# wang-q/gams

Measured on AMD Instinct MI355X. Metric: GC windows/s (size 100, step 10), higher is better.
Workload: dtype u8; 1 GPU; Atha-shaped synthetic genome (119667750 bp, piece 500000): wave size 100 step 10 lag 100 threshold 3 influence 1, peaks compacted on device; 3 batch(es) resident per GPU, steps rotate over them; batches_per_gpu=3, resident_bytes_per_gpu=358913250, passes_in_flight=3, tapered_launches=off in the timed region (passes in flight), clock_ramp_steps=4992, device=gfx950:sramecc+:xnack-, parallelism=ctg-sharded x1, no collective on the data path, collectives=none (one rank)

## Files before the change

### gams_amd/_lib.py

```python
import ctypes as C
import os

import numpy as np

_HERE = os.path.dirname(os.path.abspath(__file__))
SO_PATH = os.path.join(_HERE, "libgams_gpu.so")

OK, EINVAL, ENODEV, ENOMEM, EHIP, ESHORT, EUNSUPPORTED, ESTATE = range(8)
WAVE_PEAKS, WAVE_DENSE = 1, 2
WAVE_INPUT_AUTO, WAVE_INPUT_BYTES, WAVE_INPUT_PLANE = 0, 1, 2
WAVE_BODY_AUTO, WAVE_BODY_WIDE, WAVE_BODY_NARROW = 0, 1, 2
GC_BODY_AUTO, GC_BODY_PORTABLE, GC_BODY_AVX2 = 0, 1, 2
SW_GC, SW_COUNT = 1, 2


class GamsError(RuntimeError):
    def __init__(self, code, msg):
        super().__init__(f"gams_gpu error {code}: {msg}")
        self.code = code


class WaveParams(C.Structure):
    _fields_ = [("size", C.c_int32), ("step", C.c_int32), ("lag", C.c_uint32),
                ("threshold", C.c_float), ("influence", C.c_float)]


class GenParams(C.Structure):
    _fields_ = [("piece", C.c_int32), ("fill", C.c_int32), ("min_len", C.c_int32)]


GEN_CTG_DTYPE = np.dtype([("chr", np.uint32), ("serial", np.uint32), ("chr_start", np.int32), ("chr_end", np.int32)])
PEAK_DTYPE = np.dtype([("ctg", np.uint32), ("window", np.uint32), ("gc_count", np.uint32),
                       ("signal", np.int32)])
SW_ROW_DTYPE = np.dtype([("feature", np.uint32), ("type", np.int32), ("distance", np.int32),
                         ("start", np.int32), ("end", np.int32), ("gc_content", np.float32),
                         ("gc_mean", np.float32), ("gc_stddev", np.float32), ("gc_cv", np.float32)])

_VP = C.c_void_p
_PP = C.POINTER(C.c_void_p)
PROTOTYPES = {
    "gams_gpu_create": (C.c_int, [C.c_int, _PP]),
    "gams_gpu_destroy": (None, [_VP]),
    "gams_gpu_last_error": (C.c_char_p, [_VP]),
    "gams_gpu_device_info": (C.c_int, [_VP, C.c_char_p, C.c_size_t, C.POINTER(C.c_int32), C.POINTER(C.c_uint64)]),
    "gams_gpu_release_cached": (C.c_int, [_VP, _VP]),
    "gams_gpu_sync": (C.c_int, [_VP]),
    "gams_gpu_timer_start": (C.c_int, [_VP]),
    "gams_gpu_timer_stop": (C.c_int, [_VP, C.POINTER(C.c_float)]),
    "gams_gpu_last_kernel_ms": (C.c_int, [_VP, C.POINTER(C.c_float)]),
    "gams_gpu_last_stage_ms": (C.c_int, [_VP, _VP, C.c_uint32, C.POINTER(C.c_uint32)]),
    "gams_gpu_host_alloc": (C.c_int, [_VP, C.c_uint64, _PP]),
    "gams_gpu_host_free": (None, [_VP, _VP]),
    "gams_window_count": (C.c_int64, [C.c_int64, C.c_int32, C.c_int32]),
    "gams_seqset_create": (C.c_int, [_VP, C.c_uint32, _VP, _PP]),
    "gams_seqset_upload": (C.c_int, [_VP, _VP, C.c_uint32, _VP]),
    "gams_seqset_upload_all": (C.c_int, [_VP, _VP, _VP]),
    "gams_seqset_layout": (C.c_int, [_VP, _VP, _VP, C.POINTER(C.c_uint64)]),
    "gams_seqset_upload_image": (C.c_int, [_VP, _VP, _VP, C.c_uint64, C.c_uint64]),
    "gams_seqset_upload_ranges": (C.c_int, [_VP, _VP, _VP, _VP, C.c_uint64, C.c_uint64]),
    "gams_gc_plane": (C.c_int, [_VP, C.c_uint64, _VP]),
    "gams_gc_plane_with": (C.c_int, [_VP, C.c_uint64, _VP, C.c_int]),
    "gams_wave_plan_set_input": (C.c_int, [_VP, _VP, C.c_int]),
    "gams_wave_plan_last_input": (C.c_int, [_VP, _VP, C.POINTER(C.c_int)]),
    "gams_wave_plan_set_body": (C.c_int, [_VP, _VP, C.c_int]),
    "gams_wave_plan_last_body": (C.c_int, [_VP, _VP, C.POINTER(C.c_int)]),
    "gams_seqset_download": (C.c_int, [_VP, _VP, C.c_uint32, _VP, _VP]),
    "gams_seqset_destroy": (None, [_VP, _VP]),
    "gams_wave_plan_create": (C.c_int, [_VP, _VP, C.POINTER(WaveParams), C.c_uint32, _PP]),
    "gams_wave_plan_destroy": (None, [_VP, _VP]),
    "gams_wave_total_windows": (C.c_uint64, [_VP]),
    "gams_wave_ctg_windows": (C.c_uint32, [_VP, C.c_uint32]),
    "gams_wave_run_n": (C.c_int, [_VP, _VP, C.c_uint32]),
    "gams_wave_plan_set_depth": (C.c_int, [_VP, _VP, C.c_uint32]),
    "gams_wave_plan_select": (C.c_int, [_VP, _VP, C.c_uint32]),
    "gams_wave_plan_set_lane": (C.c_int, [_VP, _VP, C.c_uint32]),
    "gams_wave_plan_set_taper": (C.c_int, [_VP, _VP, C.c_int]),
    "gams_wave_plan_set_taper_shape": (C.c_int, [_VP, _VP, C.c_int, C.c_int]),
    "gams_wave_plan_set_queue_threads": (C.c_int, [_VP, _VP, C.c_uint32]),
    "gams_wave_plan_kernel_name": (C.c_int, [_VP, _VP, C.c_char_p, C.c_size_t]),
    "gams_wave_plan_set_pipelined": (C.c_int, [_VP, _VP, C.c_int]),
    "gams_wave_run": (C.c_int, [_VP, _VP]),
    "gams_wave_peaks": (C.c_int, [_VP, _VP, _PP, C.POINTER(C.c_uint64)]),
    "gams_wave_rows_setup": (C.c_int, [_VP, _VP, C.POINTER(C.c_char_p), _VP, C.c_float]),
    "gams_wave_rows_begin": (C.c_int, [_VP, _VP]),
    "gams_wave_rows_end": (C.c_int, [_VP, _VP, _PP, C.POINTER(C.c_uint64), _PP]),
    "gams_wave_signal_text": (C.c_int, [_VP, _VP, C.POINTER(C.c_char_p), _VP, _PP, C.POINTER(C.c_uint64), _PP]),
    "gams_wave_dense": (C.c_int, [_VP, _VP, C.c_uint32, _VP, _VP]),
    "gams_wave_plan_set_tile": (C.c_int, [_VP, _VP, C.c_uint32]),
    "gams_wave_plan_set_threads": (C.c_int, [_VP, _VP, C.c_uint32]),
    "gams_wave_plan_settled": (C.c_int, [_VP, _VP, C.POINTER(C.c_uint32), C.POINTER(C.c_int)]),
    "gams_wave_exact_count": (C.c_int, [_VP, _VP, C.POINTER(C.c_uint64)]),
    "gams_wave_plan_set_guard": (C.c_int, [_VP, _VP, C.c_float, C.c_int]),
    "gams_wave_plan_set_stamps": (C.c_int, [_VP, _VP, C.c_int]),
    "gams_wave_stamps": (C.c_int, [_VP, _VP, C.POINTER(C.c_double), C.POINTER(C.c_uint64)]),
    "gams_wave_stamps_raw": (C.c_int, [_VP, _VP, _VP, C.c_uint64]),
    "gams_gpu_wave": (C.c_int, [_VP, _VP, C.c_uint32, C.POINTER(WaveParams), _VP, _VP, C.POINTER(C.c_uint32)]),
    "gams_gpu_sw": (C.c_int, [_VP, _VP, C.c_uint32, C.c_int32, _VP, _VP, C.c_uint32, C.c_int32, C.c_int32,
                              C.c_int32, _VP, C.c_uint64, C.POINTER(C.c_uint64)]),
# ... 69 lines not shown
```

### gams_amd/csrc/wave.hip

```cpp

#include "common.hpp"

#include <algorithm>
#include <atomic>
#include <cmath>
#include <condition_variable>
#include <memory>
#include <mutex>
#include <thread>
#include <type_traits>

#include "wave_kernels.hpp"
#include "wave_repair.hpp"
#include "wave_rows.hpp"
#include "wave_select.hpp"

using WaveFastFn = void (*)(const WaveTile *, const uint8_t *, WaveArgs);
using WaveTileFn = void (*)(WaveArgs);
#define WAVE_X_PAIR(W, SIZE, STEP, LAG, NTH) \
    {wave_fast_kernel<W, SIZE, STEP, LAG, false, NTH>, wave_fast_kernel<W, SIZE, STEP, LAG, true, NTH>},
static const WaveFastFn kWaveFastFn[kWaveFastCount][2] = {WAVE_FAST_INSTANCES(WAVE_X_PAIR)};
#undef WAVE_X_PAIR
static const WaveFastFn kWaveTaperFn[2] = {wave_fast_taper_kernel<100, 10, 100, false>, wave_fast_taper_kernel<100, 10, 100, true>};
static const WaveFastFn kWaveNarrowFn = wave_fast_narrow_kernel;
static const WaveTileFn kWaveTileFn[2][2] = {{wave_tile_kernel<uint8_t, false>, wave_tile_kernel<uint8_t, true>},
                                             {wave_tile_kernel<uint16_t, false>, wave_tile_kernel<uint16_t, true>}};


struct WaveRows {
    uint32_t dmax = 0, max_name = 0;
    Kept<uint8_t> arena;
    RowTabsDev tabs;
    unsigned long long *d_words = nullptr;
    Kept<uint8_t> tmp;
    uint64_t cap = 0;
    Kept<char> d_text;
    Kept<char> h_text{true};
    Kept<unsigned long long> h_words{true};
    uint64_t copy_bytes = 0;
    bool use_graph = true;
    struct RowGraphKey {
        const void *dense, *tmp, *text, *h_text, *peaks, *tile_cnt, *tile_off;
        uint64_t dense_cap, cap, copy_bytes;
        uint32_t tile_cap, nt;
    };
    struct RowGraph {
        hipGraphExec_t exec = nullptr;
        RowGraphKey key{};
    } graph[gams_gpu::kMaxWays];
    uint64_t copied = 0;
    uint64_t last_bytes = 0;
    hipEvent_t done = nullptr;
    bool begun = false;
    void release(gams_gpu_t *h) { gams_free_all(h, arena, tmp, d_text, h_text, h_words); }
};

struct WaveSig {
// ... 53 lines not shown
    Way way[gams_gpu::kMaxWays];
    uint32_t depth = 1;
    uint32_t lane = 0;
    int taper_req = -1;
    int taper4_pct = 25, taper8_pct = 50;
    uint32_t queue_threads = gams_gpu::kMaxWays;
    uint32_t last_way = 0;
    uint32_t sel_age = 0;
    hipEvent_t ready = nullptr;
    Kept<gams_peak_t> h_peaks{true};
    uint32_t tile_cap = 0, tile_cap_req = 0;
    uint32_t tw_req = 0;
    uint32_t nth_req = 0;
    Kept<gams_peak_t> d_dense;
    uint64_t dense_cap() const { return d_dense.cap / sizeof(gams_peak_t); }
    uint64_t run_idx = 0;
    int8_t *d_const_sig = nullptr;
    unsigned long long *d_stamps = nullptr;
    unsigned long long *d_tile_off = nullptr;
    Kept<uint8_t> arena_fixed, arena_geom;
    bool ran = false;
    struct Launcher *launcher[gams_gpu::kMaxWays - 1] = {};
    bool pipelined = false;
    float g0 = 0, g1 = 0, g2 = 0, g3 = 0;
    float sq[6] = {0, 0, 0, 0, 0, 0};
    WaveRows *rows = nullptr;
    WaveSig *sigtext = nullptr;
    float guard_safety = 1.5f;
    bool guard_exact = false;
    int input_req = GAMS_WAVE_INPUT_AUTO;
    std::atomic<int> last_input{GAMS_WAVE_INPUT_BYTES};
    int body_req = GAMS_WAVE_BODY_AUTO;
    std::atomic<int> last_body{GAMS_WAVE_BODY_WIDE};
    void release(gams_gpu_t *h) {
        if (rows) rows->release(h);
        if (sigtext) sigtext->release(h);
        gams_free_all(h, arena_fixed, arena_geom, d_jtiles, d_dense, h_peaks);
        for (Way &w : way) w.release(h);
    }
};
static void wave_launcher_stop(gams_wave_plan_t *p);


namespace {

constexpr uint32_t kCounterRing = 128;
constexpr size_t kSlotWords = (size_t)kShards * kShardWords;
constexpr uint32_t kOffOneGroup = 32768;

struct Chain {
    hipStream_t st;
    hipGraph_t graph = nullptr;
    hipGraphNode_t last = nullptr;
    hipError_t err = hipSuccess;
    void kernel(const void *fn, unsigned grid, unsigned block, void **args) {
        if (err != hipSuccess) return;
        if (!graph) {
            err = hipLaunchKernel(fn, dim3(grid), dim3(block), args, 0, st);
            return;
        }
        hipKernelNodeParams kp{};
        kp.func = const_cast<void *>(fn);
        kp.gridDim = dim3(grid);
        kp.blockDim = dim3(block);
        kp.sharedMemBytes = 0;
        kp.kernelParams = args;
// ... 82 lines not shown
            p->tiles.push_back(WaveTile{c, w, n, 0u, p->ctgs[c].seq_off, p->ctgs[c].win_base});
    }
}

void wave_fill_tiles_tapered(gams_wave_plan_t *p, uint32_t slots) {
    const gams_wave_params_t &q = p->prm;
    const uint32_t tw12 = 256u * 12u - q.lag - 1u, tw8 = 256u * 8u - q.lag - 1u, tw4 = 256u * 4u - q.lag - 1u;
    const uint64_t T = p->total_windows;
    const int k4 = p->taper4_pct, k8 = p->taper8_pct;
    const uint64_t x4 = std::min<uint64_t>((uint64_t)slots * k4 / 100 * tw4, T * 8 / 100);
    const uint64_t y8 = std::min<uint64_t>((uint64_t)slots * k8 / 100 * tw8, T * 17 / 100);
    p->tiles.clear();
    for (uint32_t c = 0; c < p->set->n_ctg; ++c) {
        const uint32_t n = p->ctgs[c].n_win;
        const uint64_t after = T - p->ctgs[c].win_base;
        const uint32_t w_kind = after <= x4 ? 4u : after <= x4 + y8 ? 8u : 12u;
        const uint32_t tw = w_kind == 4u ? tw4 : w_kind == 8u ? tw8 : tw12;
        for (uint32_t w = 0; w < n; w += tw)
            p->tiles.push_back(WaveTile{c, w, n, w_kind, p->ctgs[c].seq_off, p->ctgs[c].win_base});
    }
}

int wave_build_geometry(gams_gpu_t *h, gams_wave_plan_t *p, uint32_t tw_req) {
    const WaveSelectIn in{p->prm,  p->flags,   p->serial,    p->repair, p->depth,     p->total_windows,
                          tw_req,  p->nth_req, p->taper_req, h->cus,    p->set->bytes};
    WaveSelection s;
    if (!wave_select(in, s)) return gams_fail(h, GAMS_ESTATE, "wave: the instance list lacks the selected kernel");
    p->sel = s;
    p->fast_fn = s.entry < 0 ? nullptr : s.taper ? kWaveTaperFn[s.nt] : kWaveFastFn[s.entry][s.nt];
    p->tile_fn = s.family == kWaveFamTile ? kWaveTileFn[s.k16][s.wide] : nullptr;
    if (p->fast_fn) GAMS_HIP(h, gams_lds_attr(h, reinterpret_cast<const void *>(p->fast_fn), s.lds_bytes));
    if (p->tile_fn) GAMS_HIP(h, gams_lds_attr(h, reinterpret_cast<const void *>(p->tile_fn), s.lds_bytes));
    p->body = wave_select_body(in, s);
    if (p->body.narrow) GAMS_HIP(h, gams_lds_attr(h, reinterpret_cast<const void *>(kWaveNarrowFn), p->body.lds_bytes));
    if (s.taper)
        wave_fill_tiles_tapered(p, wave_slots(h->cus));
    else
        wave_fill_tiles(p);
    return GAMS_OK;
}

void wave_set_band(gams_wave_plan_t *p) {
    float g[4];
    wave_guard_band(p->prm, (double)p->guard_safety, p->guard_exact, g);
    p->g0 = g[0];
    p->g1 = g[1];
    p->g2 = g[2];
    p->g3 = g[3];
    wave_squared_band(p->prm, g, p->sq);
}

hipStream_t wave_stream(gams_gpu_t *h, const gams_wave_plan_t *p, uint32_t k) {
    const uint32_t si = (p->lane + k) % (uint32_t)gams_gpu::kMaxWays;
    return si == 0 ? h->compute : h->aux[si - 1];
}

gams_wave_plan::Way &wave_read_way(gams_wave_plan_t *p) {
    return p->way[(p->last_way + p->depth - (p->sel_age % p->depth)) % p->depth];
}
uint32_t wave_read_way_index(const gams_wave_plan_t *p) {
    return (p->last_way + p->depth - (p->sel_age % p->depth)) % p->depth;
}

int wave_sync_ways(gams_gpu_t *h, gams_wave_plan_t *p) {
    for (uint32_t k = 0; k < p->depth; ++k) GAMS_HIP(h, hipStreamSynchronize(wave_stream(h, p, k)));
    return GAMS_OK;
}
// ... 428 lines not shown
    a.tile_cap = p->tile_cap;
    a.counters = w.d_counters + kSlotWords * slot;
    a.const_sig = p->d_const_sig;
    a.stamps = p->d_stamps;
    a.tile_cnt = w.d_tile_cnt;
    a.dense_cnt = w.d_dense_cnt;
    a.dense_sig = w.d_dense_sig;
    return a;
}

static int wave_pass_on_way(gams_gpu_t *h, gams_wave_plan_t *p, uint32_t k) {
    gams_wave_plan::Way &w = p->way[k];
    hipStream_t st = wave_stream(h, p, k);
    h->reader_epoch.fetch_add(1, std::memory_order_relaxed);
    if (st == h->compute) {
        int wrc = gams_seqset_wait_uploads(h, p->set);
        if (wrc != GAMS_OK) return wrc;
    } else if (w.seen_upload != p->set->upload_gen && p->set->uploaded) {
        GAMS_HIP(h, hipStreamWaitEvent(st, p->set->uploaded, 0));
    }
    w.seen_upload = p->set->upload_gen;
    if (!w.seen_ready) {
        GAMS_HIP(h, hipStreamWaitEvent(st, p->ready, 0));
        w.seen_ready = true;
    }
    const uint32_t slot = (uint32_t)(w.runs % kCounterRing);
    if (slot == 0 && w.runs > 0)
        GAMS_HIP(h, hipMemsetAsync(w.d_counters, 0, kCounterRing * kSlotWords * sizeof(unsigned long long), st));
    ++w.runs;
    w.last_ring = slot;
    if (p->pipelined && !w.done) GAMS_HIP(h, hipEventCreateWithFlags(&w.done, hipEventDisableTiming));
    if (p->tiles.empty()) {
        p->last_body.store(GAMS_WAVE_BODY_WIDE, std::memory_order_relaxed);
        if (p->pipelined) GAMS_HIP(h, hipEventRecord(w.done, st));
        return GAMS_OK;
    }
    const gams_wave_params_t &q = p->prm;
    const bool fast_tile = p->fast_fn != nullptr;
    const bool plane_fit = fast_tile && p->set->plane_ok && p->set->d_plane != nullptr;
    if (p->input_req == GAMS_WAVE_INPUT_PLANE && !plane_fit)
        return gams_fail(h, GAMS_ESTATE, fast_tile ? "wave: the seqset's G/C plane is stale" : "wave: this plan's kernels read the sequence bytes, not the G/C plane");
    const bool use_plane = plane_fit && (p->input_req != GAMS_WAVE_INPUT_BYTES || !p->set->have_bytes);
    if (!use_plane && !p->set->have_bytes)
        return gams_fail(h, GAMS_ESTATE, "wave: the seqset holds the G/C plane only and this plan needs the sequence bytes");
    if (p->input_req == GAMS_WAVE_INPUT_BYTES && use_plane)
        return gams_fail(h, GAMS_ESTATE, "wave: the seqset holds the G/C plane only, the bytes were asked for");
    p->last_input.store(use_plane ? GAMS_WAVE_INPUT_PLANE : GAMS_WAVE_INPUT_BYTES, std::memory_order_relaxed);
    const bool narrow_fit = use_plane && p->body.narrow;
    if (p->body_req == GAMS_WAVE_BODY_NARROW && !narrow_fit)
        return gams_fail(h, GAMS_ESTATE, p->body.narrow ? "wave: the narrow body reads the G/C plane, this pass reads the bytes"
                                                        : "wave: this plan has no narrow body");
    const bool narrow = narrow_fit && p->body_req != GAMS_WAVE_BODY_WIDE;
    p->last_body.store(narrow ? GAMS_WAVE_BODY_NARROW : GAMS_WAVE_BODY_WIDE, std::memory_order_relaxed);
    const WaveArgs a = wave_args(p, w, slot, use_plane);
    const unsigned nt = (unsigned)p->tiles.size();
    if (p->sel.direct) {
        const uint64_t total = p->total_windows;
        const unsigned blocks = (unsigned)((total + 255) / 256);
        hipLaunchKernelGGL(wave_direct_count_kernel, dim3(blocks), dim3(256), 0, st, p->set->d_seq, p->d_ctgs,
                           p->set->n_ctg, total, (uint32_t)q.size, (uint32_t)q.step, w.d_dense_cnt);
        GAMS_HIP(h, hipGetLastError());
        if (!p->serial || p->repair) {
            hipLaunchKernelGGL(wave_direct_signal_kernel, dim3(blocks), dim3(256), 0, st, p->d_ctgs, p->set->n_ctg,
                               total, w.d_dense_cnt, w.d_dense_sig, q.lag, q.threshold, (float)q.size,
                               q.lag < 2 ? 1u : 0u);
            GAMS_HIP(h, hipGetLastError());
        }
    } else if (narrow) {
        hipLaunchKernelGGL(kWaveNarrowFn, dim3(nt), dim3(p->body.nth), p->body.lds_bytes, st, a.tiles, a.seq, a);
        GAMS_HIP(h, hipGetLastError());
    } else if (p->fast_fn) {
        hipLaunchKernelGGL(p->fast_fn, dim3(nt), dim3(p->sel.nth), p->sel.lds_bytes, st, a.tiles, a.seq, a);
        GAMS_HIP(h, hipGetLastError());
    } else {
        hipLaunchKernelGGL(p->tile_fn, dim3(nt), dim3(256), p->sel.lds_bytes, st, a);
        GAMS_HIP(h, hipGetLastError());
    }
    int rc = GAMS_OK;
    if (p->sel.direct && !p->serial) {
        rc = wave_compact_dense(h, p, k, st);
        if (rc != GAMS_OK) return rc;
    }
    if (p->repair) {
        w.jac_sweeps = 0;
        w.jac_settled = false;
        w.jac_serial = false;
        rc = wave_jac_sweeps(h, p, k, kJacFirstBatch, true);
        if (rc != GAMS_OK) return rc;
    } else if (p->serial) {
        rc = wave_serial_recurrence(h, p, k, st, w.d_filtered);
        if (rc == GAMS_OK) rc = wave_compact_dense(h, p, k, st);
        if (rc != GAMS_OK) return rc;
    }
    if (p->pipelined) GAMS_HIP(h, hipEventRecord(w.done, st));
    return GAMS_OK;
}

static int wave_wait_last_run(gams_gpu_t *h, gams_wave_plan_t *p) {
    gams_wave_plan::Way &w = wave_read_way(p);
    if (p->pipelined && w.done)
        GAMS_HIP(h, hipEventSynchronize(w.done));
    else
        GAMS_HIP(h, hipStreamSynchronize(wave_stream(h, p, wave_read_way_index(p))));
    return GAMS_OK;
}

int gams_wave_plan_set_input(gams_gpu_t *h, gams_wave_plan_t *p, int mode) {
    if (!h || !p) return gams_fail(h, GAMS_EINVAL, "wave_plan_set_input: null argument");
    if (mode != GAMS_WAVE_INPUT_AUTO && mode != GAMS_WAVE_INPUT_BYTES && mode != GAMS_WAVE_INPUT_PLANE)
        return gams_fail(h, GAMS_EINVAL, "wave_plan_set_input: mode is 0 (auto), 1 (bytes) or 2 (plane)");
    p->input_req = mode;
    return GAMS_OK;
}

int gams_wave_plan_last_input(gams_gpu_t *h, gams_wave_plan_t *p, int *input) {
    if (!h || !p || !input) return gams_fail(h, GAMS_EINVAL, "wave_plan_last_input: null argument");
    if (!p->ran) return gams_fail(h, GAMS_ESTATE, "wave_plan_last_input: no run yet");
    *input = p->last_input.load(std::memory_order_relaxed);
    return GAMS_OK;
}

int gams_wave_plan_set_body(gams_gpu_t *h, gams_wave_plan_t *p, int mode) {
    if (!h || !p) return gams_fail(h, GAMS_EINVAL, "wave_plan_set_body: null argument");
    if (mode != GAMS_WAVE_BODY_AUTO && mode != GAMS_WAVE_BODY_WIDE && mode != GAMS_WAVE_BODY_NARROW)
        return gams_fail(h, GAMS_EINVAL, "wave_plan_set_body: mode is 0 (auto), 1 (wide) or 2 (narrow)");
    p->body_req = mode;
    return GAMS_OK;
}

int gams_wave_plan_last_body(gams_gpu_t *h, gams_wave_plan_t *p, int *body) {
    if (!h || !p || !body) return gams_fail(h, GAMS_EINVAL, "wave_plan_last_body: null argument");
    if (!p->ran) return gams_fail(h, GAMS_ESTATE, "wave_plan_last_body: no run yet");
    *body = p->last_body.load(std::memory_order_relaxed);
    return GAMS_OK;
}

int gams_wave_plan_set_pipelined(gams_gpu_t *h, gams_wave_plan_t *p, int enable) {
    if (!h || !p) return gams_fail(h, GAMS_EINVAL, "wave_plan_set_pipelined: null argument");
    p->pipelined = enable != 0;
    return GAMS_OK;
}

int gams_wave_run(gams_gpu_t *h, gams_wave_plan_t *p) {
    if (!h || !p) return gams_fail(h, GAMS_EINVAL, "wave_run: null argument");
    GAMS_HIP(h, hipSetDevice(h->device));
    const uint32_t k = (uint32_t)(p->run_idx % p->depth);
    int rc = wave_pass_on_way(h, p, k);
    if (rc != GAMS_OK) return rc;
    ++p->run_idx;
    p->last_way = k;
    p->sel_age = 0;
    p->ran = true;
    return GAMS_OK;
}

struct Launcher {
    std::thread th;
    std::mutex mu;
    std::condition_variable cv;
    bool armed = false, quit = false, finished = true;
    std::atomic<int> go{0};
    gams_gpu_t *h = nullptr;
    gams_wave_plan_t *p = nullptr;
    uint64_t first = 0;
    uint32_t rest = 0;
    uint32_t share = 0, shares = 1;
// ... 792 lines not shown
```

### gams_amd/csrc/wave_kernels.hpp

```cpp
#pragma once

#include "common.hpp"

#include <type_traits>

namespace {

struct WaveCtgDev {
    uint64_t seq_off;
    uint64_t win_base;
    uint32_t len;
    uint32_t n_win;
};

struct WaveTile {
    uint32_t ctg;
    uint32_t w0;
    uint32_t n_win;
    uint32_t pad;
    uint64_t seq_off;
    uint64_t win_base;
};

constexpr uint32_t kShards = 128;
// ... 855 lines not shown
template <int W, int SIZE, int STEP, int LAG, bool NT, int NTH = 256>
__device__ __forceinline__ void wave_fast_pick(const WaveTile tl, const uint8_t *const seq_p, const WaveArgs &a) {
    if (a.plane != nullptr)
        wave_fast_tile<W, SIZE, STEP, LAG, NT, NTH, true>(tl, seq_p, a);
    else
        wave_fast_tile<W, SIZE, STEP, LAG, NT, NTH, false>(tl, seq_p, a);
}

template <int W, int SIZE, int STEP, int LAG, bool NT, int NTH = 256>
__global__ __launch_bounds__(NTH, 8) void wave_fast_kernel(const WaveTile *const tiles_p, const uint8_t *const seq_p,
                                                           const WaveArgs a) {
    const WaveTile tl = tiles_p[blockIdx.x];
    wave_fast_pick<W, SIZE, STEP, LAG, NT, NTH>(tl, seq_p, a);
}

template <int SIZE, int STEP, int LAG, bool NT>
__global__ __launch_bounds__(256, 8) void wave_fast_taper_kernel(const WaveTile *const tiles_p,
                                                                 const uint8_t *const seq_p, const WaveArgs a) {
    const WaveTile tl = tiles_p[blockIdx.x];
    if (tl.pad == 12u)
        wave_fast_pick<12, SIZE, STEP, LAG, NT>(tl, seq_p, a);
    else if (tl.pad == 8u)
        wave_fast_pick<8, SIZE, STEP, LAG, NT>(tl, seq_p, a);
    else
        wave_fast_pick<4, SIZE, STEP, LAG, NT>(tl, seq_p, a);
}

__global__ __launch_bounds__(128, 8) void wave_fast_narrow_kernel(const WaveTile *const tiles_p, const uint8_t *const seq_p,
                                                                  const WaveArgs a) {
    const WaveTile tl = tiles_p[blockIdx.x];
    wave_fast_tile<24, 100, 10, 100, false, 128, true>(tl, seq_p, a);
}

__device__ __forceinline__ uint32_t wave_ctg_of(const WaveCtgDev *ctgs, uint32_t n_ctg, uint64_t g) {
    uint32_t lo = 0, hi = n_ctg;
    while (hi - lo > 1u) {
        const uint32_t mid = (lo + hi) >> 1;
        if (ctgs[mid].win_base <= g)
            lo = mid;
        else
            hi = mid;
    }
    return lo;
}

__global__ __launch_bounds__(256) void wave_direct_count_kernel(const uint8_t *seq, const WaveCtgDev *ctgs,
                                                                 uint32_t n_ctg, uint64_t total, uint32_t size,
                                                                 uint32_t step, uint32_t *dense_cnt) {
    const uint64_t g = (uint64_t)blockIdx.x * 256u + threadIdx.x;
    if (g >= total) return;
    const WaveCtgDev cg = ctgs[wave_ctg_of(ctgs, n_ctg, g)];
    const uint64_t b0 = cg.seq_off + (g - cg.win_base) * (uint64_t)step, b1 = b0 + size;
    uint32_t cnt = 0;
    for (uint64_t a = b0 & ~(uint64_t)3; a < b1; a += 4) {
        uint32_t f = gc_flags(*reinterpret_cast<const uint32_t *>(seq + a));
        if (a < b0) f &= ~0u << (8u * (uint32_t)(b0 - a));
        if (a + 4 > b1) f &= ~0u >> (8u * (uint32_t)(a + 4 - b1));
        cnt += (uint32_t)__popc(f);
    }
    dense_cnt[g] = cnt;
}

__global__ __launch_bounds__(256) void wave_direct_signal_kernel(const WaveCtgDev *ctgs, uint32_t n_ctg,
                                                                  uint64_t total, const uint32_t *dense_cnt,
                                                                  int8_t *dense_sig, uint32_t lag, float thr,
                                                                  float fsize, uint32_t no_signal) {
// ... 310 lines not shown
```

### gams_amd/csrc/wave_select.hpp

```cpp
#pragma once

#include <algorithm>
#include <cmath>
#include <cstddef>
#include <cstdint>
#include <cstdio>

#include "../../include/gams_gpu.h"

namespace {

#define WAVE_FAST_INSTANCES(X)                                                                        \
    X(20, 0, 0, 0, 256) X(12, 0, 0, 0, 256) X(8, 0, 0, 0, 256) X(4, 0, 0, 0, 256)                     \
    X(28, 100, 1, 100, 64) X(28, 100, 1, 100, 128) X(28, 100, 1, 100, 256)                            \
    X(20, 100, 1, 100, 256) X(12, 100, 1, 100, 256)                                                   \
    X(12, 100, 10, 100, 64) X(12, 100, 10, 100, 128) X(12, 100, 10, 100, 256)                         \
    X(8, 100, 10, 100, 256) X(4, 100, 10, 100, 256)                                                   \
    X(4, 100, 5, 0, 256) X(8, 100, 5, 0, 256) X(12, 100, 5, 0, 256)                                   \
    X(4, 100, 10, 0, 256) X(8, 100, 10, 0, 256) X(12, 100, 10, 0, 256)                                \
    X(4, 100, 20, 0, 256) X(8, 100, 20, 0, 256) X(12, 100, 20, 0, 256)                                \
    X(20, 100, 1, 0, 256)                                                                             \
    X(20, 100, 5, 0, 64) X(20, 100, 5, 0, 128) X(20, 100, 5, 0, 256)                                  \
    X(28, 100, 1, 0, 64) X(28, 100, 1, 0, 128) X(28, 100, 1, 0, 256)

// ... 171 lines not shown
    out.family = kWaveFamTile;
    out.tw = tw;
    out.max_win = tw + q.lag + 1;
    out.max_chunks = (uint32_t)((halo_bytes + (uint64_t)tw * q.step + 15) / 16) + 1;
    out.k16 = q.size > 255;
    const uint64_t ns = (uint64_t)q.lag * (uint64_t)q.size;
    const uint64_t q2max = (uint64_t)(out.max_win + 1) * (uint64_t)q.size * (uint64_t)q.size;
    out.wide = !(ns <= 65535 && q2max < (1ull << 32));
    out.lds_bytes = wave_lds_bytes(out.max_chunks, out.max_win, out.wide, out.k16);
    if (out.lds_bytes > 160 * 1024) return go_direct();
    return true;
}

struct WaveBody {
    bool narrow = false;
    uint32_t nth = 0, w = 0;
    size_t lds_bytes = 0;
};
constexpr int kWaveNarrowW = 24, kWaveNarrowNth = 128;

inline WaveBody wave_select_body(const WaveSelectIn &in, const WaveSelection &sel) {
    WaveBody b;
    if (sel.family != kWaveFamFast || sel.entry < 0 || sel.taper) return b;
    const WaveInstance &e = kWaveFast[sel.entry];
    if (!(e.w == 12 && e.size == 100 && e.step == 10 && e.lag == 100 && e.nth == 256)) return b;
    if ((in.flags & GAMS_WAVE_DENSE) || in.serial || in.nth_req != 0) return b;
    b.narrow = true;
    b.nth = (uint32_t)kWaveNarrowNth;
    b.w = (uint32_t)kWaveNarrowW;
    b.lds_bytes = wave_fast_lds_bytes(sel.max_chunks, b.w, (uint32_t)e.lag, false, b.nth);
    return b;
}

inline void wave_selection_name(const WaveSelection &s, char *buf, size_t n) {
    const char *nt = s.nt ? "true" : "false";
    if (s.direct)
        std::snprintf(buf, n, "wave_direct_count_kernel + wave_direct_signal_kernel");
    else if (s.taper)
        std::snprintf(buf, n, "wave_fast_taper_kernel<100, 10, 100, %s>", nt);
    else if (s.entry >= 0) {
        const WaveInstance &e = kWaveFast[s.entry];
        std::snprintf(buf, n, "wave_fast_kernel<%d, %d, %d, %d, %s, %d>", e.w, e.size, e.step, e.lag, nt, e.nth);
    } else
        std::snprintf(buf, n, "wave_tile_kernel<%s, %s>", s.k16 ? "unsigned short" : "unsigned char", s.wide ? "true" : "false");
}

}
```

### gams_amd/engine.py

```python
import ctypes as C

import numpy as np

from . import _lib
from ._lib import GamsError, WaveParams, PEAK_DTYPE, SW_ROW_DTYPE, WAVE_PEAKS, WAVE_DENSE


def _u8(buf):
    if isinstance(buf, np.ndarray):
        return np.ascontiguousarray(buf, dtype=np.uint8)
    return np.frombuffer(buf, dtype=np.uint8)


class Engine:

    def __init__(self, device=0, lib=None):
        self.lib = lib if lib is not None else _lib.load()
        h = C.c_void_p()
        rc = self.lib.gams_gpu_create(device, C.byref(h))
        if rc != _lib.OK:
            raise GamsError(rc, "gams_gpu_create failed (no HIP device?)")
        self.h = h
        self.device = device

# ... 245 lines not shown
            return int(nb.value)
        offs = np.frombuffer((C.c_uint64 * (n + 1)).from_address(off.value), np.uint64).copy()
        return (C.string_at(txt.value, nb.value) if nb.value else b""), offs

    def set_taper_shape(self, pct4, pct8=None):
        if pct8 is None:
            pct4, pct8 = divmod(int(pct4), 1000)
        self.eng.check(self.eng.lib.gams_wave_plan_set_taper_shape(self.eng.h, self.p, pct4, pct8))

    def set_queue_threads(self, n):
        self.eng.check(self.eng.lib.gams_wave_plan_set_queue_threads(self.eng.h, self.p, n))

    def kernel_name(self):
        buf = C.create_string_buffer(160)
        self.eng.check(self.eng.lib.gams_wave_plan_kernel_name(self.eng.h, self.p, buf, len(buf)))
        return buf.value.decode()

    def set_input(self, mode):
        self.eng.check(self.eng.lib.gams_wave_plan_set_input(self.eng.h, self.p, mode))

    def last_input(self):
        v = C.c_int()
        self.eng.check(self.eng.lib.gams_wave_plan_last_input(self.eng.h, self.p, C.byref(v)))
        return int(v.value)

    def set_body(self, mode):
        self.eng.check(self.eng.lib.gams_wave_plan_set_body(self.eng.h, self.p, mode))

    def last_body(self):
        v = C.c_int()
        self.eng.check(self.eng.lib.gams_wave_plan_last_body(self.eng.h, self.p, C.byref(v)))
        return int(v.value)

    def select(self, age):
        self.eng.check(self.eng.lib.gams_wave_plan_select(self.eng.h, self.p, age))

    def run_n(self, n):
        self.eng.check(self.eng.lib.gams_wave_run_n(self.eng.h, self.p, n))

    def run(self):
        self.eng.check(self.eng.lib.gams_wave_run(self.eng.h, self.p))

    def peaks(self):
        ptr, n = C.c_void_p(), C.c_uint64()
        self.eng.check(self.eng.lib.gams_wave_peaks(self.eng.h, self.p, C.byref(ptr), C.byref(n)))
        if n.value == 0:
            return np.zeros(0, PEAK_DTYPE)
        buf = (C.c_char * (n.value * PEAK_DTYPE.itemsize)).from_address(ptr.value)
        return np.frombuffer(buf, dtype=PEAK_DTYPE).copy()

    def dense(self, i):
        n = self.ctg_windows(i)
        cnt = np.zeros(max(n, 1), np.uint32)
        sig = np.zeros(max(n, 1), np.int8)
        self.eng.check(self.eng.lib.gams_wave_dense(self.eng.h, self.p, i, cnt.ctypes.data, sig.ctypes.data))
        return cnt[:n], sig[:n]

    def stamps(self):
        self.eng.check(self.eng.lib.gams_wave_plan_set_stamps(self.eng.h, self.p, 1))
        self.run()
        m = (C.c_double * 8)()
        span = C.c_uint64()
        self.eng.check(self.eng.lib.gams_wave_stamps(self.eng.h, self.p, m, C.byref(span)))
        self.eng.check(self.eng.lib.gams_wave_plan_set_stamps(self.eng.h, self.p, 0))
        span_ticks, sum_ticks = span.value >> 32, (span.value & 0xffffffff) * 16
        info = dict(clock_ghz=m[7], span_us=span_ticks / 100.0,
# ... 22 lines not shown
```

### include/gams_gpu_diag.h

```cpp
#ifndef GAMS_GPU_DIAG_H
#define GAMS_GPU_DIAG_H

#include "gams_gpu.h"

#ifdef __cplusplus
extern "C" {
#endif

int gams_gpu_timer_start(gams_gpu_t *h);
int gams_gpu_timer_stop(gams_gpu_t *h, float *ms);
int gams_gpu_last_kernel_ms(gams_gpu_t *h, float *ms);

int gams_gpu_last_stage_ms(gams_gpu_t *h, float *ms, uint32_t cap, uint32_t *n);

int gams_wave_plan_set_taper(gams_gpu_t *h, gams_wave_plan_t *plan, int mode);
int gams_wave_plan_set_taper_shape(gams_gpu_t *h, gams_wave_plan_t *plan, int pct4, int pct8);
int gams_wave_plan_set_queue_threads(gams_gpu_t *h, gams_wave_plan_t *plan, uint32_t n);
int gams_wave_plan_kernel_name(gams_gpu_t *h, gams_wave_plan_t *plan, char *buf, size_t n);
int gams_wave_plan_settled(gams_gpu_t *h, gams_wave_plan_t *plan, uint32_t *sweeps, int *serial);

int gams_wave_plan_set_tile(gams_gpu_t *h, gams_wave_plan_t *p, uint32_t tile_windows);
int gams_wave_plan_set_threads(gams_gpu_t *h, gams_wave_plan_t *p, uint32_t threads);
int gams_wave_exact_count(gams_gpu_t *h, gams_wave_plan_t *p, uint64_t *n_exact);
int gams_wave_plan_set_guard(gams_gpu_t *h, gams_wave_plan_t *p, float safety, int all_exact);
int gams_wave_plan_set_stamps(gams_gpu_t *h, gams_wave_plan_t *p, int enable);
int gams_wave_stamps(gams_gpu_t *h, gams_wave_plan_t *p, double *mean_cycles ,
                     uint64_t *span_cycles);
int gams_wave_stamps_raw(gams_gpu_t *h, gams_wave_plan_t *p, uint64_t *out, uint64_t n_words);

#define GAMS_WAVE_INPUT_AUTO 0
#define GAMS_WAVE_INPUT_BYTES 1
#define GAMS_WAVE_INPUT_PLANE 2
int gams_wave_plan_set_input(gams_gpu_t *h, gams_wave_plan_t *p, int mode);
int gams_wave_plan_last_input(gams_gpu_t *h, gams_wave_plan_t *p, int *input);
#define GAMS_WAVE_BODY_AUTO 0
#define GAMS_WAVE_BODY_WIDE 1
#define GAMS_WAVE_BODY_NARROW 2
int gams_wave_plan_set_body(gams_gpu_t *h, gams_wave_plan_t *p, int mode);
int gams_wave_plan_last_body(gams_gpu_t *h, gams_wave_plan_t *p, int *body);
#define GAMS_GC_BODY_AUTO 0
#define GAMS_GC_BODY_PORTABLE 1
#define GAMS_GC_BODY_AVX2 2
int gams_gc_plane_with(const uint8_t *seq, uint64_t n, uint8_t *plane, int body);

#ifdef __cplusplus
}
#endif
#endif
```

Baseline: 1427 billion windows/s.

## Add a one-wavefront narrow wave kernel and make it the default cut

Adds a new narrow-body kernel that runs each tile with a single 64-thread wavefront. Each thread owns 48 windows, and the lag sums are built from per-thread partial sums held in LDS. Plan setup and launch now choose between the existing two-wave narrow kernel and this cut, with one-wave as the auto default. The aim is to cut block-level synchronisation and cross-wave overhead, and to raise the number of resident blocks per CU. The cost is more serial work per thread. The tile width the kernel assumes must also match the geometry the plan already built.

Result: faster. 1557 billion windows/s (median of 6 runs) (+9.1%).

```diff
diff --git a/gams_amd/_lib.py b/gams_amd/_lib.py
--- a/gams_amd/_lib.py
+++ b/gams_amd/_lib.py
@@ -10,6 +10,7 @@
 WAVE_PEAKS, WAVE_DENSE = 1, 2
 WAVE_INPUT_AUTO, WAVE_INPUT_BYTES, WAVE_INPUT_PLANE = 0, 1, 2
 WAVE_BODY_AUTO, WAVE_BODY_WIDE, WAVE_BODY_NARROW = 0, 1, 2
+WAVE_CUT_AUTO, WAVE_CUT_TWO_WAVES, WAVE_CUT_ONE_WAVE = 0, 1, 2
 GC_BODY_AUTO, GC_BODY_PORTABLE, GC_BODY_AVX2 = 0, 1, 2
 SW_GC, SW_COUNT = 1, 2
 
@@ -64,6 +65,8 @@
     "gams_wave_plan_last_input": (C.c_int, [_VP, _VP, C.POINTER(C.c_int)]),
     "gams_wave_plan_set_body": (C.c_int, [_VP, _VP, C.c_int]),
     "gams_wave_plan_last_body": (C.c_int, [_VP, _VP, C.POINTER(C.c_int)]),
+    "gams_wave_plan_set_cut": (C.c_int, [_VP, _VP, C.c_int]),
+    "gams_wave_plan_last_cut": (C.c_int, [_VP, _VP, C.POINTER(C.c_int)]),
     "gams_seqset_download": (C.c_int, [_VP, _VP, C.c_uint32, _VP, _VP]),
     "gams_seqset_destroy": (None, [_VP, _VP]),
     "gams_wave_plan_create": (C.c_int, [_VP, _VP, C.POINTER(WaveParams), C.c_uint32, _PP]),
diff --git a/gams_amd/csrc/wave.hip b/gams_amd/csrc/wave.hip
--- a/gams_amd/csrc/wave.hip
+++ b/gams_amd/csrc/wave.hip
@@ -23,6 +23,10 @@
 #undef WAVE_X_PAIR
 static const WaveFastFn kWaveTaperFn[2] = {wave_fast_taper_kernel<100, 10, 100, false>, wave_fast_taper_kernel<100, 10, 100, true>};
 static const WaveFastFn kWaveNarrowFn = wave_fast_narrow_kernel;
+static const WaveFastFn kWaveOneWaveFn = wave_fast_onewave_kernel;
+static_assert(kOneWaveLds == wave_onewave_lds_bytes() && kOneWavePad == kWaveOneWavePad, "the one-wave carve of wave_select.hpp is the kernel's");
+static_assert(kWaveCutAuto == GAMS_WAVE_CUT_AUTO && kWaveCutTwoWaves == GAMS_WAVE_CUT_TWO_WAVES && kWaveCutOneWave == GAMS_WAVE_CUT_ONE_WAVE,
+              "wave_select.hpp names the cuts as gams_gpu_diag.h does");
 static const WaveTileFn kWaveTileFn[2][2] = {{wave_tile_kernel<uint8_t, false>, wave_tile_kernel<uint8_t, true>},
                                              {wave_tile_kernel<uint16_t, false>, wave_tile_kernel<uint16_t, true>}};
 
@@ -142,6 +146,8 @@
     std::atomic<int> last_input{GAMS_WAVE_INPUT_BYTES};
     int body_req = GAMS_WAVE_BODY_AUTO;
     std::atomic<int> last_body{GAMS_WAVE_BODY_WIDE};
+    int cut_req = GAMS_WAVE_CUT_AUTO;
+    std::atomic<int> last_cut{GAMS_WAVE_CUT_AUTO};
     void release(gams_gpu_t *h) {
         if (rows) rows->release(h);
         if (sigtext) sigtext->release(h);
@@ -290,7 +296,10 @@
     if (p->fast_fn) GAMS_HIP(h, gams_lds_attr(h, reinterpret_cast<const void *>(p->fast_fn), s.lds_bytes));
     if (p->tile_fn) GAMS_HIP(h, gams_lds_attr(h, reinterpret_cast<const void *>(p->tile_fn), s.lds_bytes));
     p->body = wave_select_body(in, s);
-    if (p->body.narrow) GAMS_HIP(h, gams_lds_attr(h, reinterpret_cast<const void *>(kWaveNarrowFn), p->body.lds_bytes));
+    if (p->body.narrow) {
+        GAMS_HIP(h, gams_lds_attr(h, reinterpret_cast<const void *>(kWaveNarrowFn), p->body.lds_bytes));
+        GAMS_HIP(h, gams_lds_attr(h, reinterpret_cast<const void *>(kWaveOneWaveFn), wave_onewave_lds_bytes()));
+    }
     if (s.taper)
         wave_fill_tiles_tapered(p, wave_slots(h->cus));
     else
@@ -785,6 +794,7 @@
     if (p->pipelined && !w.done) GAMS_HIP(h, hipEventCreateWithFlags(&w.done, hipEventDisableTiming));
     if (p->tiles.empty()) {
         p->last_body.store(GAMS_WAVE_BODY_WIDE, std::memory_order_relaxed);
+        p->last_cut.store(GAMS_WAVE_CUT_AUTO, std::memory_order_relaxed);
         if (p->pipelined) GAMS_HIP(h, hipEventRecord(w.done, st));
         return GAMS_OK;
     }
@@ -805,6 +815,11 @@
                                                         : "wave: this plan has no narrow body");
     const bool narrow = narrow_fit && p->body_req != GAMS_WAVE_BODY_WIDE;
     p->last_body.store(narrow ? GAMS_WAVE_BODY_NARROW : GAMS_WAVE_BODY_WIDE, std::memory_order_relaxed);
+    if (p->cut_req == GAMS_WAVE_CUT_ONE_WAVE && !narrow_fit)
+        return gams_fail(h, GAMS_ESTATE, p->body.narrow ? "wave: the one-wave cut reads the G/C plane, this pass reads the bytes"
+                                                        : "wave: this plan has no narrow body to cut");
+    const WaveCut cut = narrow ? wave_select_cut(p->body, p->cut_req) : WaveCut{};
+    p->last_cut.store(cut.cut, std::memory_order_relaxed);
     const WaveArgs a = wave_args(p, w, slot, use_plane);
     const unsigned nt = (unsigned)p->tiles.size();
     if (p->sel.direct) {
@@ -820,7 +835,8 @@
             GAMS_HIP(h, hipGetLastError());
         }
     } else if (narrow) {
-        hipLaunchKernelGGL(kWaveNarrowFn, dim3(nt), dim3(p->body.nth), p->body.lds_bytes, st, a.tiles, a.seq, a);
+        const WaveFastFn cut_fn = cut.cut == GAMS_WAVE_CUT_ONE_WAVE ? kWaveOneWaveFn : kWaveNarrowFn;
+        hipLaunchKernelGGL(cut_fn, dim3(nt), dim3(cut.nth), cut.lds_bytes, st, a.tiles, a.seq, a);
         GAMS_HIP(h, hipGetLastError());
     } else if (p->fast_fn) {
         hipLaunchKernelGGL(p->fast_fn, dim3(nt), dim3(p->sel.nth), p->sel.lds_bytes, st, a.tiles, a.seq, a);
@@ -885,6 +901,21 @@
     if (!h || !p || !body) return gams_fail(h, GAMS_EINVAL, "wave_plan_last_body: null argument");
     if (!p->ran) return gams_fail(h, GAMS_ESTATE, "wave_plan_last_body: no run yet");
     *body = p->last_body.load(std::memory_order_relaxed);
+    return GAMS_OK;
+}
+
+int gams_wave_plan_set_cut(gams_gpu_t *h, gams_wave_plan_t *p, int mode) {
+    if (!h || !p) return gams_fail(h, GAMS_EINVAL, "wave_plan_set_cut: null argument");
+    if (mode != GAMS_WAVE_CUT_AUTO && mode != GAMS_WAVE_CUT_TWO_WAVES && mode != GAMS_WAVE_CUT_ONE_WAVE)
+        return gams_fail(h, GAMS_EINVAL, "wave_plan_set_cut: mode is 0 (auto), 1 (two waves) or 2 (one wave)");
+    p->cut_req = mode;
+    return GAMS_OK;
+}
+
+int gams_wave_plan_last_cut(gams_gpu_t *h, gams_wave_plan_t *p, int *cut) {
+    if (!h || !p || !cut) return gams_fail(h, GAMS_EINVAL, "wave_plan_last_cut: null argument");
+    if (!p->ran) return gams_fail(h, GAMS_ESTATE, "wave_plan_last_cut: no run yet");
+    *cut = p->last_cut.load(std::memory_order_relaxed);
     return GAMS_OK;
 }
 
diff --git a/gams_amd/csrc/wave_kernels.hpp b/gams_amd/csrc/wave_kernels.hpp
--- a/gams_amd/csrc/wave_kernels.hpp
+++ b/gams_amd/csrc/wave_kernels.hpp
@@ -911,6 +911,281 @@
     wave_fast_tile<24, 100, 10, 100, false, 128, true>(tl, seq_p, a);
 }
 
+constexpr uint32_t kOneWavePad = 128;
+constexpr uint32_t kOneWavePieces = (((64u * 48u * 10u + 100u + 30u) / 16u + 1u) + 7u + 7u) / 8u;
+constexpr uint32_t kOneWaveLds = kOneWavePad + kOneWavePieces * 16u + (64u + 16u) * 8u;
+__device__ __forceinline__ void wave_onewave_tile(const WaveTile tl, const uint8_t *const seq_p, const WaveArgs &a) {
+    constexpr uint32_t W = 48, HW = 24, NT_ = 64, SIZE = 100, STEP = 10, LAG = 100;
+    constexpr uint32_t TW = NT_ * W - LAG - 1u;
+    constexpr uint32_t PAD = kOneWavePad, NV = kOneWavePieces;
+    static_assert(NV == (((NT_ * W * STEP + SIZE + 30u) / 16u + 1u) + 7u + 7u) / 8u, "the pieces of wave_fast_tile's plane copy");
+    constexpr uint32_t NLV = (NV + NT_ - 1u) / NT_;
+    constexpr uint32_t NBITS = W * STEP + SIZE;
+    constexpr uint32_t NDW = (NBITS + 31u) / 32u + 1u;
+    constexpr uint32_t OVER = PAD + NV * 16u;
+    static_assert(PAD * 8u >= (LAG + 1u) * STEP, "the pad holds every bit in front of a ctg start");
+    static_assert(((PAD * 8u + 127u + (NT_ - 1u) * W * STEP) >> 5) + NDW <= OVER / 4u, "phase 2 reads inside pad | BM");
+    static_assert((NT_ - 1u) * W + LAG + W + 8u <= OVER, "K (with the slots masked threads read) fits under pad | BM");
+    static_assert(LAG / W == 2u && LAG % W == 4u && W % 8u == 0u, "lag sums: two PS blocks + the dword at K byte 48 t + 96, a qword's first");
+    extern __shared__ __align__(16) unsigned char smem[];
+    const uint32_t *BW = reinterpret_cast<const uint32_t *>(smem);
+    uint8_t *K = smem;
+    uint2 *PS = reinterpret_cast<uint2 *>(smem + OVER);
+
+    const uint32_t tid = threadIdx.x;
+    if (a.stamps != nullptr && tid == 0) a.stamps[(size_t)blockIdx.x * 16 + 10] = __builtin_amdgcn_s_memrealtime();
+    const uint32_t lag = LAG;
+    const uint32_t w0 = tl.w0;
+    const uint32_t w1 = min(w0 + TW, tl.n_win);
+    const uint32_t nvalid = w1 - w0;
+    const int32_t vb = (int32_t)w0 - (int32_t)LAG - 1;
+    const uint32_t wh = vb > 0 ? (uint32_t)vb : 0u;
+    const uint32_t a0 = (wh * STEP) & ~127u;
+
+    wave_stamp(a, 0);
+    {
+        const uint4 *const pl = reinterpret_cast<const uint4 *>(a.plane + ((tl.seq_off + a0) >> 3));
+        uint4 *const BV = reinterpret_cast<uint4 *>(smem + PAD);
+        uint4 v[NLV];
+#pragma unroll
+        for (uint32_t k = 0; k < NLV; ++k) v[k] = pl[min(tid + NT_ * k, NV - 1u)];
+        if (tid < PAD / 16u) reinterpret_cast<uint4 *>(smem)[tid] = make_uint4(0u, 0u, 0u, 0u);
+#pragma unroll
+        for (uint32_t k = 0; k < NLV; ++k) BV[min(tid + NT_ * k, NV - 1u)] = v[k];
+    }
+    __syncthreads();
+    wave_stamp(a, 1);
+    wave_stamp(a, 2);
+
+    const uint32_t nK = LAG + 1u + nvalid;
+    const uint32_t base = tid * W;
+    uint32_t r[NDW];
+    {
+        const uint32_t x0 = (uint32_t)((vb + (int32_t)base) * (int32_t)STEP - (int32_t)a0 + (int32_t)(PAD * 8u));
+        const uint32_t d0 = x0 >> 5, sh = x0 & 31u;
+#pragma unroll
+        for (uint32_t i = 0; i < NDW; ++i) r[i] = BW[d0 + i];
+#pragma unroll
+        for (uint32_t i = 0; i + 1u < NDW; ++i) r[i] = __builtin_amdgcn_alignbit(r[i + 1u], r[i], sh);
+    }
+    __syncthreads();
+    if (base < nK) {
+        auto field = [&](uint32_t off) -> uint32_t {
+            const uint32_t d = off >> 5, s = off & 31u;
+            if (s + STEP <= 32u) return __builtin_amdgcn_ubfe(r[d], s, STEP);
+            return __builtin_amdgcn_alignbit(r[d + 1u], r[d], s) & ((1u << STEP) - 1u);
+        };
+        uint32_t k = 0;
+#pragma unroll
+        for (uint32_t d = 0; d < SIZE / 32u; ++d) k += __popc(r[d]);
+        k += __popc(r[SIZE / 32u] & ((1u << (SIZE % 32u)) - 1u));
+        uint32_t packed = k, held = 0, s1 = 0, s2 = 0;
+        auto put = [&](uint32_t j4, uint32_t four) {
+            s1 = __builtin_amdgcn_udot4(four, 0x01010101u, s1, false);
+            s2 = __builtin_amdgcn_udot4(four, four, s2, false);
+            if ((j4 & 4u) == 0u)
+                held = four;
+            else if (base + j4 - 4u < nK)
+                reinterpret_cast<uint2 *>(K)[(base + j4 - 4u) >> 3] = make_uint2(held, four);
+        };
+#pragma unroll
+        for (uint32_t j = 1; j < W; ++j) {
+            k += __popc(field(SIZE + (j - 1u) * STEP));
+            k -= __popc(field((j - 1u) * STEP));
+            if ((j & 3u) == 0u) {
+                put(j - 4u, packed);
+                packed = k;
+            } else {
+                packed |= k << (8u * (j & 3u));
+            }
+        }
+        put(W - 4u, packed);
+        PS[tid] = make_uint2(s1, s2);
+    }
+    if (vb < 0) {
+        __syncthreads();
+        const uint32_t nz = (uint32_t)(-vb);
+        if (base < nz) {
+            uint32_t *const KT = reinterpret_cast<uint32_t *>(K) + (base >> 2);
+            uint32_t s1 = 0, s2 = 0;
+#pragma unroll
+            for (uint32_t d = 0; d < W / 4u; ++d) {
+                uint32_t x = KT[d];
+                const uint32_t j4 = base + 4u * d;
+                if (nz > j4) x = nz >= j4 + 4u ? 0u : x & (~0u << (8u * (nz - j4)));
+                KT[d] = x;
+                s1 = __builtin_amdgcn_udot4(x, 0x01010101u, s1, false);
+                s2 = __builtin_amdgcn_udot4(x, x, s2, false);
+            }
+            PS[tid] = make_uint2(s1, s2);
+        }
+    }
+    __syncthreads();
+    wave_stamp(a, 3);
+
+    uint64_t crest = 0, trough = 0, pend = 0;
+    {
+        const uint2 *const K2 = reinterpret_cast<const uint2 *>(K) + tid * (W / 8u);
+        uint64_t can = 0;
+        if (!a.no_signal && base < nvalid) {
+            const uint32_t hi_q = min(W, nvalid - base);
+            const uint32_t lo_q = w0 + base >= lag ? 0u : min(W, lag - (w0 + base));
+            can = ((1ull << hi_q) - 1ull) & ~((1ull << lo_q) - 1ull);
+        }
+        const float nf = (float)LAG, aA = a.aA, aB = a.aB;
+        float S1f = 0.0f, S2f = 0.0f, kinf = 0.0f;
+        uint64_t sig64 = 0, nos64 = 0, dn64 = 0;
+#pragma unroll
+        for (uint32_t run = 0; run < 2u; ++run) {
+            uint32_t og[HW / 4u], kq[8];
+            if (run != 0u) __builtin_amdgcn_sched_barrier(0);
+#pragma unroll
+            for (uint32_t d = 0; d < 3u; ++d) {
+                const uint2 t = K2[3u * run + d];
+                og[2u * d] = t.x;
+                og[2u * d + 1u] = t.y;
+            }
+#pragma unroll
+            for (uint32_t d = 0; d < 4u; ++d) {
+                const uint2 t = K2[12u + 3u * run + d];
+                kq[2u * d] = t.x;
+                kq[2u * d + 1u] = t.y;
+            }
+            if (run == 0u) {
+                const uint2 p0 = PS[tid], p1 = PS[tid + 1u];
+                uint32_t S1 = p0.x + p1.x, S2 = p0.y + p1.y;
+                S1 = __builtin_amdgcn_udot4(kq[0], 0x01010101u, S1, false);
+                S2 = __builtin_amdgcn_udot4(kq[0], kq[0], S2, false);
+                S1f = (float)S1;
+                S2f = (float)S2;
+                kinf = (float)(kq[1] & 0xFFu);
+            }
+            uint32_t sigm = 0, nosm = 0, dnm = 0;
+            float cA = 0.0f, cB = 0.0f;
+#pragma unroll
+            for (uint32_t q = 0; q < HW; ++q) {
+                if (q % 12u == 0u) {
+                    const float ub = S1f + (float)(12u * SIZE);
+                    cA = __builtin_fmaf(a.gA1, ub, a.gA0);
+                    cB = __builtin_fmaf(a.gB1, ub, a.gB0);
+                }
+                const float koutf = (float)((og[q >> 2] >> (8u * (q & 3u))) & 0xFFu);
+                const float kkf = (float)((kq[1u + ((q + 1u) >> 2)] >> (8u * ((q + 1u) & 3u))) & 0xFFu);
+                uint32_t xs, xn, dn;
+                z_decide(nf, kkf, S1f, S2f, aA, aB, cA, cB, xs, xn, dn);
+                sigm = __builtin_amdgcn_alignbit(sigm, xs, 31);
+                nosm = __builtin_amdgcn_alignbit(nosm, xn, 31);
+                dnm = __builtin_amdgcn_alignbit(dnm, dn, 31);
+                S1f = (S1f - koutf) + kinf;
+                S2f = __builtin_fmaf(-koutf, koutf, S2f);
+                S2f = __builtin_fmaf(kinf, kinf, S2f);
+                kinf = kkf;
+            }
+            sig64 |= (uint64_t)(__brev(sigm) >> (32u - HW)) << (HW * run);
+            nos64 |= (uint64_t)(__brev(nosm) >> (32u - HW)) << (HW * run);
+            dn64 |= (uint64_t)(__brev(dnm) >> (32u - HW)) << (HW * run);
+        }
+        if (!(a.g0 < INFINITY)) sig64 = nos64 = 0;
+        uint64_t decided = sig64 | nos64;
+        crest = sig64 & ~dn64;
+        trough = sig64 & dn64;
+        const uint32_t qlag = lag - (w0 + base);
+        if (qlag < W) {
+            const uint64_t bit = 1ull << qlag;
+            uint32_t s1 = 0, s2 = 0;
+            for (uint32_t j = 0; j < lag; ++j) {
+                const uint32_t kv = K[base + qlag + 1u + j];
+                s1 += kv;
+                s2 += kv * kv;
+            }
+            const uint32_t kk = K[base + qlag + lag + 1u];
+            uint32_t xs, xn, dn;
+            z_decide(nf, (float)kk, (float)s1, (float)s2, aA, aB, __builtin_fmaf(a.gA1, (float)s1, a.gA0),
+                     __builtin_fmaf(a.gB1, (float)s1, a.gB0), xs, xn, dn);
+            const bool sg = (xs >> 31) != 0u, no = (xn >> 31) != 0u, below = (dn >> 31) != 0u;
+            const bool exact_all = !(a.g0 < INFINITY);
+            decided = ((sg || no) && !exact_all) ? (decided | bit) : (decided & ~bit);
+            crest = (sg && !below) ? (crest | bit) : (crest & ~bit);
+            trough = (sg && below) ? (trough | bit) : (trough & ~bit);
+        }
+        crest &= can & decided;
+        trough &= can & decided;
+        pend = can & ~decided;
+        if (__ballot(pend != 0ull)) {
+            uint64_t todo = pend;
+            while (todo) {
+                const uint32_t q = (uint32_t)__ffsll((unsigned long long)todo) - 1u;
+                todo &= todo - 1ull;
+                const uint32_t i = w0 + base + q;
+                const uint32_t tj = base + q + (i == lag ? 1u : 0u);
+                const uint32_t kk = K[base + q + lag + 1u];
+                bool same = true;
+                for (uint32_t j = 0; j < lag && same; ++j) same = K[tj + j] == kk;
+                if (same) {
+                    const int sg = a.const_sig[kk];
+                    pend &= ~(1ull << q);
+                    crest |= sg > 0 ? 1ull << q : 0ull;
+                    trough |= sg < 0 ? 1ull << q : 0ull;
+                }
+            }
+        }
+    }
+    wave_stamp(a, 4);
+    {
+        unsigned long long bal = __ballot(pend != 0ull);
+        uint32_t n_exact = 0;
+        while (bal) {
+            const int L = __ffsll(bal) - 1;
+            const uint32_t plo = (uint32_t)__builtin_amdgcn_readlane((int)(uint32_t)pend, L);
+            const uint32_t phi = (uint32_t)__builtin_amdgcn_readlane((int)(uint32_t)(pend >> 32), L);
+            const uint32_t q = plo ? (uint32_t)__ffs((int)plo) - 1u : 31u + (uint32_t)__ffs((int)phi);
+            const uint32_t baseL = (uint32_t)L * W;
+            const uint32_t first = (w0 + baseL + q == lag) ? 1u : 0u;
+            const int sg = exact_signal_wave(K, baseL + q + first, baseL + q + lag + 1u, lag, a.fsize, a.thr);
+            if (tid == (uint32_t)L) {
+                pend &= ~(1ull << q);
+                crest |= sg > 0 ? 1ull << q : 0ull;
+                trough |= sg < 0 ? 1ull << q : 0ull;
+            }
+            ++n_exact;
+            bal = __ballot(pend != 0ull);
+        }
+        if (n_exact && tid == 0)
+            atomicAdd(&a.counters[(blockIdx.x & (kShards - 1u)) * kShardWords + 1u], (unsigned long long)n_exact);
+    }
+    wave_stamp(a, 5);
+    if ((a.flags & GAMS_WAVE_PEAKS) != 0) {
+        const uint64_t both = crest | trough;
+        const uint32_t mine = (uint32_t)__popcll((unsigned long long)both);
+        gams_peak_t *const region = a.peaks + (size_t)blockIdx.x * a.tile_cap;
+        const uint32_t inc = wave_incl_scan(mine);
+        const uint32_t tot = (uint32_t)__builtin_amdgcn_readlane((int)inc, 63);
+        if (tid == 0) a.tile_cnt[blockIdx.x] = tot;
+        uint32_t pos = inc - mine;
+        uint64_t bits = both;
+        while (bits) {
+            const uint32_t q = (uint32_t)__ffsll((unsigned long long)bits) - 1u;
+            bits &= bits - 1ull;
+            if (pos < a.tile_cap) {
+                gams_peak_t pk;
+                pk.ctg = tl.ctg;
+                pk.window = w0 + base + q;
+                pk.gc_count = K[base + q + lag + 1u];
+                pk.signal = ((crest >> q) & 1ull) ? 1 : -1;
+                region[pos] = pk;
+            }
+            ++pos;
+        }
+    }
+    wave_stamp(a, 6);
+}
+
+__global__ __launch_bounds__(64, 8) void wave_fast_onewave_kernel(const WaveTile *const tiles_p, const uint8_t *const seq_p,
+                                                                  const WaveArgs a) {
+    const WaveTile tl = tiles_p[blockIdx.x];
+    wave_onewave_tile(tl, seq_p, a);
+}
+
 __device__ __forceinline__ uint32_t wave_ctg_of(const WaveCtgDev *ctgs, uint32_t n_ctg, uint64_t g) {
     uint32_t lo = 0, hi = n_ctg;
     while (hi - lo > 1u) {
diff --git a/gams_amd/csrc/wave_select.hpp b/gams_amd/csrc/wave_select.hpp
--- a/gams_amd/csrc/wave_select.hpp
+++ b/gams_amd/csrc/wave_select.hpp
@@ -227,6 +227,39 @@
     return b;
 }
 
+enum : int { kWaveCutAuto = 0, kWaveCutTwoWaves = 1, kWaveCutOneWave = 2 };
+struct WaveCut {
+    int cut = 0;
+    uint32_t nth = 0, w = 0;
+    size_t lds_bytes = 0;
+};
+constexpr int kWaveOneWaveW = 48, kWaveOneWaveNth = 64;
+constexpr int kWaveCutDefault = kWaveCutOneWave;
+constexpr uint32_t kWaveOneWavePad = 128;
+
+constexpr size_t wave_onewave_bm_bytes() {
+    const uint32_t chunks = ((uint32_t)(kWaveOneWaveNth * kWaveOneWaveW) * 10u + 100u + 30u) / 16u + 1u;
+    return kWaveOneWavePad + (size_t)((chunks + 7u + 7u) / 8u) * 16u;
+}
+constexpr size_t wave_onewave_k_bytes() { return (size_t)(kWaveOneWaveNth - 1) * kWaveOneWaveW + 152u; }
+constexpr size_t wave_onewave_lds_bytes() { return wave_onewave_bm_bytes() + (size_t)(kWaveOneWaveNth + 16) * 8u; }
+
+inline WaveCut wave_select_cut(const WaveBody &body, int cut_req) {
+    WaveCut c;
+    if (!body.narrow) return c;
+    c.cut = cut_req == kWaveCutAuto ? kWaveCutDefault : cut_req;
+    if (c.cut == kWaveCutOneWave) {
+        c.nth = (uint32_t)kWaveOneWaveNth;
+        c.w = (uint32_t)kWaveOneWaveW;
+        c.lds_bytes = wave_onewave_lds_bytes();
+    } else {
+        c.nth = body.nth;
+        c.w = body.w;
+        c.lds_bytes = body.lds_bytes;
+    }
+    return c;
+}
+
 inline void wave_selection_name(const WaveSelection &s, char *buf, size_t n) {
     const char *nt = s.nt ? "true" : "false";
     if (s.direct)
diff --git a/gams_amd/engine.py b/gams_amd/engine.py
--- a/gams_amd/engine.py
+++ b/gams_amd/engine.py
@@ -301,6 +301,14 @@
         self.eng.check(self.eng.lib.gams_wave_plan_last_body(self.eng.h, self.p, C.byref(v)))
         return int(v.value)
 
+    def set_cut(self, mode):
+        self.eng.check(self.eng.lib.gams_wave_plan_set_cut(self.eng.h, self.p, mode))
+
+    def last_cut(self):
+        v = C.c_int()
+        self.eng.check(self.eng.lib.gams_wave_plan_last_cut(self.eng.h, self.p, C.byref(v)))
+        return int(v.value)
+
     def select(self, age):
         self.eng.check(self.eng.lib.gams_wave_plan_select(self.eng.h, self.p, age))
 
diff --git a/include/gams_gpu_diag.h b/include/gams_gpu_diag.h
--- a/include/gams_gpu_diag.h
+++ b/include/gams_gpu_diag.h
@@ -38,6 +38,11 @@
 #define GAMS_WAVE_BODY_NARROW 2
 int gams_wave_plan_set_body(gams_gpu_t *h, gams_wave_plan_t *p, int mode);
 int gams_wave_plan_last_body(gams_gpu_t *h, gams_wave_plan_t *p, int *body);
+#define GAMS_WAVE_CUT_AUTO 0
+#define GAMS_WAVE_CUT_TWO_WAVES 1
+#define GAMS_WAVE_CUT_ONE_WAVE 2
+int gams_wave_plan_set_cut(gams_gpu_t *h, gams_wave_plan_t *p, int mode);
+int gams_wave_plan_last_cut(gams_gpu_t *h, gams_wave_plan_t *p, int *cut);
 #define GAMS_GC_BODY_AUTO 0
 #define GAMS_GC_BODY_PORTABLE 1
 #define GAMS_GC_BODY_AVX2 2
```
